# FluxML/Flux3D.jl

Hardware: AMD Instinct MI355X
Metric: chamfer_point_pairs_per_sec (higher is better)
Workload: dtype f32

## Files before the change

flux3d.jl_amd/csrc/chamfer.hip:

```cpp
#include <cmath>

#include "nn1_common.h"

using namespace fx3d;

#ifdef FX3D_PROBE
__device__ unsigned long long g_probe[4096 * 16];
#define FX3D_PROBE_MARK(k)                                                                   \
    do {                                                                                     \
        if (threadIdx.x == 0 && blockIdx.x < 4096) {                                         \
            g_probe[blockIdx.x * 16 + (k)] = __builtin_readcyclecounter();                   \
            if ((k) == 0) g_probe[blockIdx.x * 16 + 13] = wall_clock64();                    \
            if ((k) == 12) g_probe[blockIdx.x * 16 + 14] = wall_clock64();                   \
        }                                                                                    \
    } while (0)
__device__ unsigned long long g_probe2[256 * 16];
#define FX3D_PROBE_MARK2(k) do { if (threadIdx.x == 0 && blockIdx.x < 256) g_probe2[blockIdx.x * 16 + (k)] = __builtin_readcyclecounter(); } while (0)
__device__ unsigned long long g_probe3[16 * 16 * 8];
#define FX3D_PROBE_MARKW(k) do { if ((threadIdx.x & 63) == 0 && blockIdx.x < 16) g_probe3[(blockIdx.x * 16 + (threadIdx.x >> 6)) * 8 + (k)] = __builtin_readcyclecounter(); } while (0)
#else
#define FX3D_PROBE_MARK(k) do { } while (0)
#define FX3D_PROBE_MARK2(k) do { } while (0)
#define FX3D_PROBE_MARKW(k) do { } while (0)
#endif
// ... 53 lines not shown
    199, 198, 134, 135, 143, 142, 206, 207, 215, 223, 159, 151, 150, 158, 222, 214, 213, 221, 220, 212, 148, 156, 157, 149, 141, 205, 204, 140, 132, 196, 197, 133,
    69, 5, 4, 68, 76, 12, 13, 77, 85, 93, 92, 84, 20, 28, 29, 21, 22, 30, 94, 86, 87, 95, 31, 23, 15, 14, 78, 79, 71, 70, 6, 7,
};
constexpr size_t kHScratchBytes = (kHThreads / 64) * (32 * 8 + kHItemCap * 2 + 32 * 3 * 4) + 64 * 32;

__device__ __forceinline__ float vmin(float a, float b) {
    float r;
    asm("v_min_f32 %0, %1, %2" : "=v"(r) : "v"(a), "v"(b));
    return r;
}

__device__ __forceinline__ void split2h(float v, _Float16 &h, _Float16 &l) {
    h = (_Float16)v;
    l = (_Float16)(v - (float)h);
}

constexpr float kBetaC = 0x1.1p-18f;
constexpr float kBandB1 = 1.0f + 18.0f * kBetaC + 0x1p-20f;
constexpr float kBandA = 22.3f * kBetaC + 0x1p-19f;
__device__ __forceinline__ void make_pieces(float cx, float cy, float cz, h8 &p0, h8 &p1) {
    _Float16 hx, lx, hy, ly, hz, lz, n1, n2, n3;
    split2h(cx, hx, lx); split2h(cy, hy, ly); split2h(cz, hz, lz);
    const float n0 = ((cx * cx) + (cy * cy)) + (cz * cz);
    const float n = n0 + kBetaC * n0;
    n1 = (_Float16)n;
    const float r1 = n - (float)n1;
    n2 = (_Float16)r1;
    n3 = (_Float16)(r1 - (float)n2);
    const _Float16 z = (_Float16)0.0f;
    p0 = h8{hx, hx, lx, hy, hy, ly, hz, hz};
    p1 = h8{lz, n1, n2, n3, lx, ly, lz, z};
}

template <bool WANT_IDX, bool SPLITFUSE = false, bool PRUNE = false>
__global__ __launch_bounds__(kHThreads, 4) void nn1_f16_kernel(Nn1Params p) {
    extern __shared__ __attribute__((aligned(16))) float lds[];
    __shared__ __attribute__((aligned(16))) float red[4 * 4 * (kHThreads / 64) + 16];
    __shared__ int nfar[2];
    __shared__ unsigned short farlist[kHFarCap];
    constexpr int QB = (kHThreads / 64) * 32;

    const int L = blockIdx.x;
    const int per_cloud = p.tiles * p.nsplit;
    const bool by_xcd = 2 * p.B >= 8;
    const int slot = by_xcd ? L >> 3 : L;
    const int c = by_xcd ? (slot / per_cloud) * 8 + (L & 7) : slot / per_cloud;
    const int tile = (slot % per_cloud) / p.nsplit;
    const int split = (slot % per_cloud) % p.nsplit;
    if (c >= 2 * p.B) return;
    const int dir = c >= p.B ? 1 : 0;
    const int b = dir ? c - p.B : c;
    const int NQ = dir ? p.M : p.N;
    const int NC = dir ? p.N : p.M;
    if (tile >= (dir ? p.tiles_y : p.tiles_x)) return;
    if ((long long)split * p.chunk >= NC) return;
    const int ctail = (p.tail > 0 && p.nsplit == 1 && NC > p.chunk && NC - p.chunk <= p.tail) ? NC - p.chunk : 0;
    const int NCm = NC - ctail;
    const float *__restrict__ qb = (dir ? p.y : p.x) + (size_t)b * NQ * 3;
    const float *__restrict__ cb = (dir ? p.x : p.y) + (size_t)b * NC * 3;
    int32_t *idx_out = dir ? p.idx_y : p.idx_x;
    float *dmin_out = dir ? p.dmin_y : p.dmin_x;

    const int tid = threadIdx.x, lane = tid & 63;
    const int wv = __builtin_amdgcn_readfirstlane(tid >> 6);
    const int jq = lane & 31, hh = lane >> 5;
    const int CH = p.chunk;
    const int tpb = dir ? p.tpb_y : p.tpb;
    h8 *imgp = reinterpret_cast<h8 *>(lds);
    float4 *imgf = reinterpret_cast<float4 *>(lds);
    unsigned long long *wres = reinterpret_cast<unsigned long long *>(lds + 8 * (CH + 64));
    unsigned short *witems = reinterpret_cast<unsigned short *>(wres + (kHThreads / 64) * 32);
    float *wq = reinterpret_cast<float *>(witems + (kHThreads / 64) * kHItemCap);
    unsigned long long *qres = wres + wv * 32;
    unsigned short *items = witems + wv * kHItemCap;
    float *qtab = wq + wv * 96;
    const bool vec = (reinterpret_cast<uintptr_t>(cb) & 15) == 0;
    const bool one_shot = NCm <= CH;
    if (tid == 0) { nfar[0] = 0; nfar[1] = 0; }
    float qpre[3];
    {
        const int q0i = (tile * tpb) * QB + wv * 32 + jq;
        const int qc0 = q0i < NQ ? q0i : NQ - 1;
#pragma unroll
        for (int d = 0; d < 3; ++d) qpre[d] = qb[(size_t)qc0 * 3 + d];
    }
    if constexpr (PRUNE) {
        unsigned int *zc = reinterpret_cast<unsigned int *>(wres);
        for (int i = tid; i < 1040 + 16 * 256; i += kHThreads) zc[i] = 0u;
        int *gb = reinterpret_cast<int *>(wq + (kHThreads / 64) * 96) + 64 * 8;
        for (int i = tid; i < kHGroupsMax * 8; i += kHThreads) gb[i] = (i & 4) ? (int)0x80000000 : 0x7fffffff;
    }
    FX3D_PROBE_MARK(0);

    const bool own_chunk_only = p.nsplit > 1 && (long long)split * CH + (long long)p.nsplit * CH >= NCm;
    const int s_lo = own_chunk_only ? split * CH : 0;
    const int SN = own_chunk_only ? (NCm - s_lo < CH ? NCm - s_lo : CH) : NC;
    const float *__restrict__ sb = cb + (size_t)s_lo * 3;
    const bool parked = one_shot || own_chunk_only;
    float mu[3], cinf = 0.0f, varmax = 0.0f;
    float bxlo[3] = {0.f, 0.f, 0.f}, bxhi[3] = {0.f, 0.f, 0.f};
    bool allfin = true;
    {
        float mn[3] = {INFINITY, INFINITY, INFINITY}, mx[3] = {-INFINITY, -INFINITY, -INFINITY}, sm3[3] = {0.f, 0.f, 0.f};
        float sqt = 0.0f;
        const float pil[3] = {sb[0], sb[1], sb[2]};
        const int nsweep = (SN + kHThreads - 1) / kHThreads;
        for (int i0 = 0; i0 < nsweep; i0 += 4) {
            P3 v[4];
#pragma unroll
            for (int e = 0; e < 4; ++e) {
                const int pt = (i0 + e) * kHThreads + tid;
                v[e] = *reinterpret_cast<const P3 *>(sb + (size_t)(pt < SN ? pt : SN - 1) * 3);
            }
#pragma unroll
            for (int e = 0; e < 4; ++e) {
                const int pt = (i0 + e) * kHThreads + tid;
                mn[0] = fminf(mn[0], v[e].x); mx[0] = fmaxf(mx[0], v[e].x);
                mn[1] = fminf(mn[1], v[e].y); mx[1] = fmaxf(mx[1], v[e].y);
                mn[2] = fminf(mn[2], v[e].z); mx[2] = fmaxf(mx[2], v[e].z);
                if (pt < SN) {
                    sm3[0] = sm3[0] + v[e].x; sm3[1] = sm3[1] + v[e].y; sm3[2] = sm3[2] + v[e].z;
                    if (parked) imgf[((pt >> 5) * 2) * 32 + (pt & 31)] = float4{v[e].x, v[e].y, v[e].z, 0.0f};
                }
// ... 33 lines not shown
#undef NN1_ROW_SUM
            const float lo3[3] = {lo4.x, lo4.y, lo4.z}, hi3[3] = {hi4.x, hi4.y, hi4.z}, st3[3] = {st4.x, st4.y, st4.z};
            float m3[3], ci = 0.0f, vm = st4.w / fmaxf(0.25f * (float)SN, 1.0f);
            bool fin = true;
#pragma unroll
            for (int d = 0; d < 3; ++d) {
                const float lo = lo3[d], hi = hi3[d], st = st3[d];
                m3[d] = fminf(fmaxf(st / (float)SN, lo), hi);
                const float off = st / (float)SN - pil[d];
                vm = vm - off * off;
                ci = fmaxf(ci, fmaxf(hi - m3[d], m3[d] - lo));
                fin = fin && fabsf(st) < INFINITY;
            }
            if (lane == 0) {
                float4 *o4 = reinterpret_cast<float4 *>(red) + 4 * (kHThreads / 64);
                o4[0] = float4{m3[0], m3[1], m3[2], ci * 1.000001f};
                o4[1] = float4{vm, fin ? 1.0f : 0.0f, 0.0f, 0.0f};
                if (PRUNE) { o4[2] = float4{lo3[0], lo3[1], lo3[2], 0.0f}; o4[3] = float4{hi3[0], hi3[1], hi3[2], 0.0f}; }
            }
        }
        __syncthreads();
        {
            const float4 *o4 = reinterpret_cast<const float4 *>(red) + 4 * (kHThreads / 64);
            const float4 a = o4[0], b2 = o4[1];
            mu[0] = a.x; mu[1] = a.y; mu[2] = a.z; cinf = a.w;
            varmax = b2.x; allfin = b2.y != 0.0f;
            if (PRUNE) {
                const float4 l4 = o4[2], h4 = o4[3];
                bxlo[0] = l4.x; bxlo[1] = l4.y; bxlo[2] = l4.z; bxhi[0] = h4.x; bxhi[1] = h4.y; bxhi[2] = h4.z;
            }
        }
    }
    float rng = cinf;
    if (allfin && cinf < 1.0e16f && 3.0f * cinf * cinf > kRobustGate * varmax) {
        const float4 r = robust_range3<kHThreads, false>(sb, SN, parked, imgf, red, mu[0], mu[1], mu[2], cinf);
        mu[0] = r.x; mu[1] = r.y; mu[2] = r.z; rng = r.w;
    }
    const bool sane = allfin && cinf < 1.0e16f;
    float sc = 1.0f;
    if (sane && rng > 1.0e-30f) {
        int e;
        (void)frexpf(rng, &e);
        sc = ldexpf(1.0f, 7 - e);
    }
    auto uni = [](float v) { return __builtin_bit_cast(float, __builtin_amdgcn_readfirstlane(__builtin_bit_cast(int, v))); };
    mu[0] = uni(mu[0]); mu[1] = uni(mu[1]); mu[2] = uni(mu[2]); sc = uni(sc); rng = uni(rng); cinf = uni(cinf);
    const bool has_far = sane && rng < cinf;
    int fslot = 0;
    auto pieces = [&](float x, float y, float z, int pt, h8 &p0, h8 &p1) {
        const float sx = (x - mu[0]) * sc, sy = (y - mu[1]) * sc, sz = (z - mu[2]) * sc;
        if (!has_far) { make_pieces(sx, sy, sz, p0, p1); return; }
        const bool far = !(fmaxf(fmaxf(fabsf(sx), fabsf(sy)), fabsf(sz)) < 128.0f);
        make_pieces(far ? 0.f : sx, far ? 0.f : sy, far ? 0.f : sz, p0, p1);
        if (far) {
            p1[7] = (_Float16)kPadF16;
            const int f = atomicAdd(&nfar[fslot], 1);
            if (f < kHFarCap) farlist[f] = (unsigned short)pt;
        }
    };

    [[maybe_unused]] float4 *cs = nullptr, *qsw = nullptr;
    [[maybe_unused]] bool sorted_c = false;
    [[maybe_unused]] int qwlen = 0;
    [[maybe_unused]] float4 *boxes = nullptr;
    if constexpr (PRUNE) {
        cs = p.pscr + (size_t)blockIdx.x * p.pscr_stride;
        qsw = cs + kHChunkMax;
        boxes = reinterpret_cast<float4 *>(wq + (kHThreads / 64) * 96);
        unsigned int *ccnt = reinterpret_cast<unsigned int *>(wres);
        unsigned int *qtot = ccnt + 520;
        unsigned int *qwh = qtot + 520;
        const bool last_t = tile == (dir ? p.tiles_y : p.tiles_x) - 1;
        const int qw0 = tile * tpb * QB;
        const int qw1 = last_t || qw0 + tpb * QB > NQ ? NQ : qw0 + tpb * QB;
        qwlen = qw1 - qw0;
        const int cnt = NCm;
        const bool do_sort = sane && cnt >= 512;
        const bool sorted_q = do_sort && NQ <= 4 * kHThreads;
        P3 qv[4];
        if (sorted_q) {
#pragma unroll
            for (int e = 0; e < 4; ++e) {
                const int qp = 256 * wv + 64 * e + lane;
                qv[e] = *reinterpret_cast<const P3 *>(qb + (size_t)(qp < NQ ? qp : NQ - 1) * 3);
            }
        }
        FX3D_PROBE_MARK2(0);
        int *gbox = reinterpret_cast<int *>(boxes + 64 * 2);
        auto group_box = [&](int wrow, float x, float y, float z) {
            int *g = gbox + (wrow >> 5) * 8;
            atomicMin(g + 0, fkey((x - mu[0]) * sc)); atomicMin(g + 1, fkey((y - mu[1]) * sc)); atomicMin(g + 2, fkey((z - mu[2]) * sc));
            atomicMax(g + 4, fkey((x - mu[0]) * sc)); atomicMax(g + 5, fkey((y - mu[1]) * sc)); atomicMax(g + 6, fkey((z - mu[2]) * sc));
        };
        if (do_sort) {
            float4 cv[4];
#pragma unroll
            for (int e = 0; e < 4; ++e) {
                const int pt = e * kHThreads + tid;
                cv[e] = float4{0.f, 0.f, 0.f, 0.f};
                if (pt < cnt) cv[e] = imgf[((pt >> 5) * 2) * 32 + (pt & 31)];
            }
            FX3D_PROBE_MARK2(1);
            float inv[3], off[3], cfl[3], cfh[3];
#pragma unroll
            for (int d = 0; d < 3; ++d) {
                const float fr = has_far ? 0.125f * rng : 128.0f / sc;
                const float flo = fmaxf(bxlo[d], mu[d] - fr), fhi = fminf(bxhi[d], mu[d] + fr);
                inv[d] = fhi > flo ? 8.0f / (fhi - flo) : 0.0f;
                off[d] = -flo * inv[d];
                cfl[d] = flo; cfh[d] = fhi;
            }
            auto cell = [&](float x, float y, float z) -> unsigned int {
                const unsigned int ux = (unsigned int)(int)fminf(fmaxf(__builtin_fmaf(x, inv[0], off[0]), 0.0f), 7.0f);
                const unsigned int uy = (unsigned int)(int)fminf(fmaxf(__builtin_fmaf(y, inv[1], off[1]), 0.0f), 7.0f);
                const unsigned int uz = (unsigned int)(int)fminf(fmaxf(__builtin_fmaf(z, inv[2], off[2]), 0.0f), 7.0f);
                return ux | (uy << 3) | (uz << 6);
            };

            unsigned int ccr[4], qcr[4];
            auto count_cells = [&](bool valid, unsigned int t, auto &&add) -> unsigned int {
                unsigned int rank = 0u;
                bool mine = valid;
                const unsigned int tn = (unsigned int)__builtin_amdgcn_update_dpp((int)~t, (int)t, 0x111, 0xF, 0xF, false);
                if (__builtin_popcountll(__ballot(valid && t == tn)) >= 8) {
                    unsigned long long rem = __ballot(valid);
                    for (int it = 0; it < 12 && rem; ++it) {
                        const unsigned int t0 = (unsigned int)__builtin_amdgcn_readlane((int)t, __builtin_ctzll(rem));
                        const unsigned long long grp = __ballot(mine && t == t0);
                        rem &= ~grp;
                        if (__builtin_popcountll(grp) < 4) continue;
                        unsigned int base = 0u;
                        if ((int)lane == __builtin_ctzll(grp)) base = add(t0, (unsigned int)__builtin_popcountll(grp));
                        base = (unsigned int)__builtin_amdgcn_readlane((int)base, __builtin_ctzll(grp));
                        if (mine && t == t0) {
                            rank = base + __builtin_amdgcn_mbcnt_hi((unsigned int)(grp >> 32), __builtin_amdgcn_mbcnt_lo((unsigned int)grp, 0u));
                            mine = false;
                        }
                    }
                }
                if (mine) rank = add(t, 1u);
                return rank;
            };
#pragma unroll
            for (int e = 0; e < 4; ++e) {
                const int pt = e * kHThreads + tid;
                const unsigned int t = pt < cnt ? cell(cv[e].x, cv[e].y, cv[e].z) : 0u;
                ccr[e] = (t << 16) | count_cells(pt < cnt, t, [&](unsigned int c, unsigned int n) { return atomicAdd(&ccnt[c], n); });
            }
            int *qbb = reinterpret_cast<int *>(boxes + 64 * 2 + kHGroupsMax * 2 - 2);
            if (sorted_q) {
                int kl[3] = {0x7fffffff, 0x7fffffff, 0x7fffffff}, kh[3] = {(int)0x80000000, (int)0x80000000, (int)0x80000000};
#pragma unroll
                for (int e = 0; e < 4; ++e) {
                    const int qp = 256 * wv + 64 * e + lane;
                    if (qp < NQ) {
                        const int k3[3] = {fkey(qv[e].x), fkey(qv[e].y), fkey(qv[e].z)};
#pragma unroll
                        for (int d = 0; d < 3; ++d) { kl[d] = kl[d] < k3[d] ? kl[d] : k3[d]; kh[d] = kh[d] > k3[d] ? kh[d] : k3[d]; }
                    }
                }
#pragma unroll
                for (int d = 0; d < 3; ++d) {
                    int a = row_mm_key<false>(kl[d]), b2 = row_mm_key<true>(kh[d]);
                    a = imm<false>(a, dpp_keepi<0x142, 0xA>(a)); a = imm<false>(a, dpp_keepi<0x143, 0xC>(a));
                    b2 = imm<true>(b2, dpp_keepi<0x142, 0xA>(b2)); b2 = imm<true>(b2, dpp_keepi<0x143, 0xC>(b2));
                    if (lane == 63) { atomicMin(qbb + d, a); atomicMax(qbb + 4 + d, b2); }
                }
            }
            FX3D_PROBE_MARK2(2);
            __syncthreads();
            FX3D_PROBE_MARK2(3);
            float qinv[3] = {0.f, 0.f, 0.f}, qoff[3] = {0.f, 0.f, 0.f};
            if (sorted_q) {
                const float ext = fmaxf(fmaxf(cfh[0] - cfl[0], cfh[1] - cfl[1]), cfh[2] - cfl[2]);
#pragma unroll
// ... 86 lines not shown
                            group_box(rank - qw0, qv[e].x, qv[e].y, qv[e].z);
                        }
                    }
                }
            }
        }
        if (!sorted_q) {
            for (int q0 = qw0 + wv * 64; q0 < qw1; q0 += kHThreads) {
                const int qp = q0 + lane;
                const P3 r = *reinterpret_cast<const P3 *>(qb + (size_t)(qp < qw1 ? qp : qw1 - 1) * 3);
                if (qp < qw1) qsw[qp - qw0] = float4{r.x, r.y, r.z, __builtin_bit_cast(float, qp)};
                const int kx = fkey((r.x - mu[0]) * sc), ky = fkey((r.y - mu[1]) * sc), kz = fkey((r.z - mu[2]) * sc);
                const int lx = row_mm_key<false>(kx), ly = row_mm_key<false>(ky), lz = row_mm_key<false>(kz);
                const int hx = row_mm_key<true>(kx), hy = row_mm_key<true>(ky), hz = row_mm_key<true>(kz);
                if ((lane & 15) == 0 && qp < qw1) {
                    int *g = gbox + ((qp - qw0) >> 5) * 8;
                    atomicMin(g + 0, lx); atomicMin(g + 1, ly); atomicMin(g + 2, lz);
                    atomicMax(g + 4, hx); atomicMax(g + 5, hy); atomicMax(g + 6, hz);
                }
            }
        }
        FX3D_PROBE_MARK2(8);
    }
    FX3D_PROBE_MARK(1);

    const float cm2 = 3.0f * (fminf(cinf * sc, 128.0f) * fminf(cinf * sc, 128.0f));
    float qr[3], da = 0.0f;
    float da_far = 0.0f;
    [[maybe_unused]] float dpr = INFINITY;
    bool qfin = true;
    int qi = 0;
    bool qok = true;
    h8 bq;
    double acc = 0.0;

    const int jfirst = split * CH, jstep = p.nsplit * CH;
    for (int j0 = jfirst; j0 < NCm; j0 += jstep) {
        const int cnt = (NCm - j0) < CH ? (NCm - j0) : CH;
        const int cnt_pad = (cnt + 32 * kHLT - 1) / (32 * kHLT) * (32 * kHLT);
        if (j0 > jfirst) __syncthreads();
        if constexpr (PRUNE) {
            for (int tl = tid >> 4; tl * 64 < cnt_pad + 64; tl += kHThreads / 16) {
                float4 r4[4];
#pragma unroll
                for (int k = 0; k < 4; ++k) {
                    const int pt = tl * 64 + k * 16 + (tid & 15);
                    r4[k] = float4{0.f, 0.f, 0.f, 0.f};
                    if (pt < cnt) r4[k] = imgf[((pt >> 5) * 2) * 32 + (pt & 31)];
                }
                float lo3[3] = {INFINITY, INFINITY, INFINITY}, hi3[3] = {-INFINITY, -INFINITY, -INFINITY};
#pragma unroll
                for (int k = 0; k < 4; ++k) {
                    const int pt = tl * 64 + k * 16 + (tid & 15), i0 = ((pt >> 5) * 2) * 32 + (pt & 31);
                    h8 p0, p1;
                    if (pt < cnt) {
                        pieces(r4[k].x, r4[k].y, r4[k].z, pt, p0, p1);
                        const int id = sorted_c ? __builtin_bit_cast(int, r4[k].w) : j0 + pt;
                        cs[pt] = float4{r4[k].x, r4[k].y, r4[k].z, __builtin_bit_cast(float, id)};
                        const float b3[3] = {(r4[k].x - mu[0]) * sc, (r4[k].y - mu[1]) * sc, (r4[k].z - mu[2]) * sc};
#pragma unroll
                        for (int d = 0; d < 3; ++d) { lo3[d] = vmin(lo3[d], b3[d]); hi3[d] = -vmin(-hi3[d], -b3[d]); }
                    } else {
                        make_pieces(0.f, 0.f, 0.f, p0, p1);
                        p1[7] = (_Float16)kPadF16;
                    }
                    imgp[i0] = p0;
                    imgp[i0 + 32] = p1;
                }
                float bl[3], bh[3];
#pragma unroll
// ... 632 lines not shown
        }
        const float dd = __builtin_bit_cast(float, (unsigned int)(r >> 32));
        int32_t *idx_out = dir ? p.idx_y : p.idx_x;
        float *dmin_out = dir ? p.dmin_y : p.dmin_x;
        if (idx_out) idx_out[(size_t)b * NQ + qi] = (int)(unsigned int)r;
        if (dmin_out) dmin_out[(size_t)b * NQ + qi] = dd;
        acc = (double)dd;
    }
    if (p.partials) {
        __shared__ double sm[kThreads / 64];
        const double tot = block_sum<kThreads>(acc, sm);
        if (!p.ticket) {
            if (threadIdx.x == 0) p.partials[(size_t)c * tiles_f + blockIdx.x] = tot;
            return;
        }
        if (threadIdx.x < 64) {
            const FinalizeArgs fa{reinterpret_cast<unsigned long long *>(p.partials), p.ticket, p.nvalid, p.B, tiles_f, p.tiles_x, p.tiles_y,
                                  p.sums_out, p.loss_out, p.N, p.M, p.Bg, p.w1, p.w2};
            (void)fused_finalize_wave0(fa, (size_t)c * tiles_f + blockIdx.x, tot, (int)threadIdx.x);
        }
    }
}

}

namespace fx3d {

size_t nn1_f16_lds_bytes(int chunk) { return (size_t)chunk * 8 * sizeof(float) + kHScratchBytes; }

constexpr size_t kHBoxBytes = 64 * 2 * sizeof(float4) + kHGroupsMax * 32;

template <bool WANT_IDX>
static fx3d_status launch_f16(const Nn1Params &p, int grid, size_t lds_bytes, hipStream_t st) {
    void (*const kfn)(Nn1Params) = p.pscr ? &nn1_f16_kernel<WANT_IDX, false, true>
                                   : p.fuse_split ? &nn1_f16_kernel<WANT_IDX, true> : &nn1_f16_kernel<WANT_IDX, false>;
    const size_t box = p.pscr ? kHBoxBytes : 0;
    const fx3d_status arc = ensure_dynamic_lds(reinterpret_cast<const void *>(kfn), (int)(nn1_f16_lds_bytes(kHChunkMax) + box), "nn1_f16_kernel");
    if (arc != FX3D_OK) return arc;
    hipLaunchKernelGGL(kfn, dim3(grid), dim3(kHThreads), lds_bytes + box, st, p);
    FX3D_LAUNCH_CHECK();
    return FX3D_OK;
}

fx3d_status nn1_f16_launch(const Nn1Params &p, int grid, size_t lds_bytes, hipStream_t st) {
    return p.idx_x || p.idx_y ? launch_f16<true>(p, grid, lds_bytes, st) : launch_f16<false>(p, grid, lds_bytes, st);
}

fx3d_status nn1_split_finalize_launch(const Nn1Params &p, int tiles_f, hipStream_t st) {
    hipLaunchKernelGGL(nn1_split_finalize_kernel, dim3(tiles_f, 2 * p.B), dim3(kThreads), 0, st, p, tiles_f);
    FX3D_LAUNCH_CHECK();
    return FX3D_OK;
}

}
```

flux3d.jl_amd/csrc/chamfer_host.hip:

```cpp
#include <cmath>
#include <cstdlib>

#include "nn1_common.h"

using namespace fx3d;

namespace {

struct FinalizeParams {
    const double *partials;
    int B, tiles, tiles_x, tiles_y;
    double *sums;
    float *loss;
    int N, M, D;
    long long Bg;
    float w1, w2;
};

__global__ __launch_bounds__(kThreads) void chamfer_finalize_partials_kernel(FinalizeParams f) {
    __shared__ double sm[kThreads / 64];
    double tot[2];
    for (int dir = 0; dir < 2; ++dir) {
        const int nt = dir ? f.tiles_y : f.tiles_x;
        const long long n = (long long)f.B * nt;
// ... 174 lines not shown
    if (plan_kernel(pl, D) != NN1_F16 || pl.nsplit != 1 || pl.tail != 0 || maxc > pl.chunk || maxc < 1024 || !opt(OPT_NN1_PRUNE)) return 0;
    if ((pl.tpb > pl.tpb_y ? pl.tpb : pl.tpb_y) * 16 + 2 > kHGroupsMax - 1) return 0;
    if ((pl.tpb < pl.tpb_y ? pl.tpb : pl.tpb_y) < 2) return 0;
    return kHChunkMax + (pl.tpb > pl.tpb_y ? pl.tpb : pl.tpb_y) * 512 + kHTail;
}

struct Workspace {
    int tiles;
    size_t sums, gres, need, pscr, total;
};
Workspace workspace_layout(const Plan &pl, int N, int M, int B, int D) {
    Workspace w{};
    const int maxq = N > M ? N : M;
    w.tiles = pl.nsplit > 1 ? ceil_div(maxq, kThreads) : pl.tiles;
    w.sums = (size_t)2 * B * w.tiles * sizeof(double);
    w.gres = w.sums + 2 * sizeof(double);
    w.need = w.gres + (pl.nsplit > 1 ? (size_t)pl.nsplit * 2 * B * maxq * sizeof(unsigned long long) : 0);
    w.pscr = (w.need + 255) & ~(size_t)255;
    const size_t ps = (size_t)prune_rows_per_block(pl, N, M, D) * pl.grid * sizeof(float4);
    w.total = ps ? w.pscr + ps : w.need;
    return w;
}

constexpr long long kSplitFuseMax = 255;

fx3d_status run_nn1(Nn1Params p, int D, const Plan &pl, hipStream_t st) {
    p.tiles = pl.tiles; p.tiles_x = pl.tiles_x; p.tiles_y = pl.tiles_y; p.chunk = pl.chunk;
    p.tpb = pl.tpb; p.tpb_y = pl.tpb_y;
    p.tail = pl.tail;
    p.nsplit = p.gres ? pl.nsplit : 1;
    p.fuse_split = p.gres && p.ticket ? 1 : 0;
    p.pscr_stride = p.pscr ? prune_rows_per_block(pl, p.N, p.M, D) : 0;
    if (!p.pscr_stride) p.pscr = nullptr;
    const Nn1Kernel k = plan_kernel(pl, D);
    ProfileScope prof("nn1", st);
    if (k == NN1_F16) return nn1_f16_launch(p, pl.grid, pl.lds_bytes, st);
    return nn1_exact_launch(k, p, D, pl.R, pl.grid, pl.lds_bytes, st);
}

}

namespace fx3d {

fx3d_status chamfer_check_shapes(const char *fn, const void *x, int N, const void *y, int M, int B, int D) {
    FX3D_REQUIRE(x && y, "%s: null input pointer", fn);
    FX3D_REQUIRE(N > 0 && M > 0 && B > 0 && D > 0, "%s: empty input (N=%d M=%d B=%d D=%d)", fn, N, M, B, D);
    FX3D_REQUIRE((long long)B * 2 * (((long long)(N > M ? N : M) + 255) / 256) < (1ll << 30),
                 "%s: problem too large for one launch", fn);
    return FX3D_OK;
}

fx3d_status chamfer_forward(const float *x, int N, const float *y, int M, int B, int D, double *sums_dev, float *loss_dev,
                            long long Bg, float w1, float w2, int32_t *idx_x, int32_t *idx_y, void *ws, size_t ws_bytes,
                            hipStream_t st, const char *fn) {
    fx3d_status rc = chamfer_check_shapes(fn, x, N, y, M, B, D);
    if (rc) return rc;
    const Plan pl = make_plan(N, M, B, D);
    const Workspace w = workspace_layout(pl, N, M, B, D);
    if (!ws || ws_bytes < w.need) {
        set_error("%s: workspace too small (%zu < %zu bytes)", fn, ws ? ws_bytes : (size_t)0, w.need);
        return FX3D_ERR_WORKSPACE;
    }
    char *const base = static_cast<char *>(ws);
    Nn1Params p{};
    p.x = x; p.y = y; p.N = N; p.M = M; p.B = B;
    p.idx_x = idx_x; p.idx_y = idx_y;
// ... 113 lines not shown
```

flux3d.jl_amd/csrc/nn1_common.h:

```cpp
#pragma once
#include "fx3d_common.h"

namespace fx3d {

constexpr int kThreads = 256;
constexpr int kTile = 32;
constexpr int kChunkMax = 4096;

struct Nn1Params {
    const float *x;
    const float *y;
    int N, M, B;
    int32_t *idx_x, *idx_y;
    float *dmin_x, *dmin_y;
    double *partials;
    int tiles;
    int tiles_x, tiles_y;
    int chunk;
    int tpb;
    int tpb_y;
    unsigned int *ticket;
    unsigned int nvalid;
    double *sums_out;
    float *loss_out;
    float w1, w2;
    long long Bg;
    int nsplit;
    unsigned long long *gres;
    int qstride;
    int fuse_split;
    int tail;
    float4 *pscr;
    int pscr_stride;
};

enum Nn1Kernel { NN1_GENERIC, NN1_SMALL_D, NN1_TINY, NN1_F16 };
fx3d_status nn1_exact_launch(Nn1Kernel k, const Nn1Params &p, int D, int R, int grid, size_t lds_bytes, hipStream_t st);
size_t nn1_f16_lds_bytes(int chunk);
fx3d_status nn1_f16_launch(const Nn1Params &p, int grid, size_t lds_bytes, hipStream_t st);
fx3d_status nn1_split_finalize_launch(const Nn1Params &p, int tiles_f, hipStream_t st);

__device__ __forceinline__ float min3f(float a, float b, float c) {
    return __builtin_fminf(__builtin_fminf(a, b), c);
}

template <int DIM>
__device__ __forceinline__ float sqd(const float (&q)[DIM], const float (&c)[DIM]) {
    float t0 = q[0] - c[0];
    float s = t0 * t0;
#pragma unroll
    for (int d = 1; d < DIM; ++d) {
        float t = q[d] - c[d];
        s = s + t * t;
    }
    return s;
}

__device__ __forceinline__ bool fless(float a, float b) { return (a < b) || (b != b && a == a); }
__device__ __forceinline__ unsigned int dist_key(float d) { return d != d ? 0x7fc00000u : __builtin_bit_cast(unsigned int, d); }

template <int DIM>
__device__ __forceinline__ void nn1_scan_isless(const float (&q)[DIM], const float *__restrict__ cb, int NC, float &best, int &bi) {
    float c0[DIM];
#pragma unroll
    for (int d = 0; d < DIM; ++d) c0[d] = cb[d];
    best = sqd<DIM>(q, c0);
    bi = 0;
    for (int j = 1; j < NC; ++j) {
        float cc[DIM];
#pragma unroll
        for (int d = 0; d < DIM; ++d) cc[d] = cb[(size_t)j * DIM + d];
        const float dd = sqd<DIM>(q, cc);
        if (fless(dd, best)) { best = dd; bi = j; }
    }
}

constexpr int kHThreads = 1024;
#ifndef FX3D_HLT
#define FX3D_HLT 2
#endif
constexpr int kHLT = FX3D_HLT;
constexpr int kHChunkMax = 4096;
constexpr int kHTail = 64;
constexpr int kHGroupsMax = 8 * 16 + 2 + 1;

constexpr int kTyThreads = 256;
constexpr int kTyQ = 16;
constexpr int kTySl = 16;
constexpr int kTyG = 16;

__device__ __forceinline__ float chamfer_loss_from_sums(double sa, double sb, int N, int M, int D,
                                                        long long Bg, float w1, float w2) {
    const float dA = (float)(sa / ((double)D * (double)N * (double)Bg)) * 3.0f;
    const float dB = (float)(sb / ((double)D * (double)M * (double)Bg)) * 3.0f;
    return (w1 * dA) + (w2 * dB);
}

#if defined(__HIP_DEVICE_COMPILE__) && !defined(__gfx950__)
#error "nn1_common.h: the relaxed-atomic + s_waitcnt hand-off between blocks is validated on gfx950 only (see the note above)"
#endif
struct FinalizeArgs {
    unsigned long long *pp;
    unsigned int *ticket;
    unsigned int nvalid;
    int B, stride, tiles_x, tiles_y;
    double *sums_out;
    float *loss_out;
    int N, M;
    long long Bg;
    float w1, w2;
};
__device__ __forceinline__ int fused_finalize_wave0(const FinalizeArgs &f, size_t slot, double tot, int lane) {
    int last = 0;
    if (lane == 0) {
        __hip_atomic_store(&f.pp[slot], __builtin_bit_cast(unsigned long long, tot), __ATOMIC_RELAXED, __HIP_MEMORY_SCOPE_AGENT);
        asm volatile("s_waitcnt vmcnt(0)" ::: "memory");
        const unsigned int old = __hip_atomic_fetch_add(f.ticket, 1u, __ATOMIC_RELAXED, __HIP_MEMORY_SCOPE_AGENT);
// ... 34 lines not shown
```

Before: 14590 billion.

## Add uniform-grid spatial hash fast path for pruned nearest-neighbor search

Adds a GRID variant of the pruned f16 kernel. For compact, well-conditioned single-chunk clouds it bins the candidate points into a G^3 uniform grid in LDS using a counting sort. Each query then searches the 27 neighboring cells, and expands rings with a provable distance bound for queries that are not yet resolved. When the grid checks fail or too many queries remain unresolved, it falls back to the existing sort/box-prune path. This trades brute-force tiled distance evaluation for data-dependent exact search, with added complexity, scalar-divergent ring loops, and extra synchronisations.

New measurement: 18920 billion (median of 6 runs). 29.7% higher.

```diff
diff --git a/flux3d.jl_amd/csrc/chamfer.hip b/flux3d.jl_amd/csrc/chamfer.hip
--- a/flux3d.jl_amd/csrc/chamfer.hip
+++ b/flux3d.jl_amd/csrc/chamfer.hip
@@ -109,12 +109,15 @@
     p1 = h8{lz, n1, n2, n3, lx, ly, lz, z};
 }
 
-template <bool WANT_IDX, bool SPLITFUSE = false, bool PRUNE = false>
+template <bool WANT_IDX, bool SPLITFUSE = false, bool PRUNE = false, bool GRID = false>
 __global__ __launch_bounds__(kHThreads, 4) void nn1_f16_kernel(Nn1Params p) {
     extern __shared__ __attribute__((aligned(16))) float lds[];
     __shared__ __attribute__((aligned(16))) float red[4 * 4 * (kHThreads / 64) + 16];
     __shared__ int nfar[2];
     __shared__ unsigned short farlist[kHFarCap];
+    __shared__ int gflag;
+    __shared__ unsigned int gocc;
+    __shared__ unsigned int gunf;
     constexpr int QB = (kHThreads / 64) * 32;
 
     const int L = blockIdx.x;
@@ -161,11 +164,22 @@
 #pragma unroll
         for (int d = 0; d < 3; ++d) qpre[d] = qb[(size_t)qc0 * 3 + d];
     }
+    [[maybe_unused]] int gG = kGridMinG;
     if constexpr (PRUNE) {
         unsigned int *zc = reinterpret_cast<unsigned int *>(wres);
         for (int i = tid; i < 1040 + 16 * 256; i += kHThreads) zc[i] = 0u;
         int *gb = reinterpret_cast<int *>(wq + (kHThreads / 64) * 96) + 64 * 8;
         for (int i = tid; i < kHGroupsMax * 8; i += kHThreads) gb[i] = (i & 4) ? (int)0x80000000 : 0x7fffffff;
+        if constexpr (GRID) if (p.grid) {
+            while (gG < kGridMaxG && kGridPpc * (gG + 1) * (gG + 1) * (gG + 1) <= NCm) ++gG;
+            unsigned int *gz = reinterpret_cast<unsigned int *>(lds) + ((NCm + 63) >> 6) * 256 + 128;
+            if (NCm >= kGridMinCand) {
+                const int i4 = 4 * tid;
+                if (i4 < gG * gG * gG + 4) *reinterpret_cast<uint4 *>(&gz[i4 + (i4 & ~127)]) = uint4{0u, 0u, 0u, 0u};
+                if (tid == 0 && gG == kGridMaxG) *reinterpret_cast<uint4 *>(&gz[2 * 4096]) = uint4{0u, 0u, 0u, 0u};
+            }
+            if (tid == 0) { gflag = 0; gocc = 0u; gunf = 0u; }
+        }
     }
     FX3D_PROBE_MARK(0);
 
@@ -265,9 +279,11 @@
         }
     }
     float rng = cinf;
+    [[maybe_unused]] bool robust_ran = false;
     if (allfin && cinf < 1.0e16f && 3.0f * cinf * cinf > kRobustGate * varmax) {
         const float4 r = robust_range3<kHThreads, false>(sb, SN, parked, imgf, red, mu[0], mu[1], mu[2], cinf);
         mu[0] = r.x; mu[1] = r.y; mu[2] = r.z; rng = r.w;
+        robust_ran = true;
     }
     const bool sane = allfin && cinf < 1.0e16f;
     float sc = 1.0f;
@@ -292,11 +308,300 @@
         }
     };
 
+    [[maybe_unused]] auto count_cells = [&](bool valid, unsigned int t, auto &&add) -> unsigned int {
+        unsigned int rank = 0u;
+        bool mine = valid;
+        const unsigned int tn = (unsigned int)__builtin_amdgcn_update_dpp((int)~t, (int)t, 0x111, 0xF, 0xF, false);
+        if (__builtin_popcountll(__ballot(valid && t == tn)) >= 8) {
+            unsigned long long rem = __ballot(valid);
+            for (int it = 0; it < 12 && rem; ++it) {
+                const unsigned int t0 = (unsigned int)__builtin_amdgcn_readlane((int)t, __builtin_ctzll(rem));
+                const unsigned long long grp = __ballot(mine && t == t0);
+                rem &= ~grp;
+                if (__builtin_popcountll(grp) < 4) continue;
+                unsigned int base = 0u;
+                if ((int)lane == __builtin_ctzll(grp)) base = add(t0, (unsigned int)__builtin_popcountll(grp));
+                base = (unsigned int)__builtin_amdgcn_readlane((int)base, __builtin_ctzll(grp));
+                if (mine && t == t0) {
+                    rank = base + __builtin_amdgcn_mbcnt_hi((unsigned int)(grp >> 32), __builtin_amdgcn_mbcnt_lo((unsigned int)grp, 0u));
+                    mine = false;
+                }
+            }
+        }
+        if (mine) rank = add(t, 1u);
+        return rank;
+    };
+    [[maybe_unused]] bool grid_done = false;
+    [[maybe_unused]] double gacc = 0.0;
+    [[maybe_unused]] float4 gcv[4];
+    [[maybe_unused]] P3 gqv[4];
+    [[maybe_unused]] bool gpre = false, gabandon = false;
+    if constexpr (PRUNE && GRID) {
+        bool gtry = p.grid && NQ <= 4 * kHThreads && sane && !has_far && !robust_ran && one_shot && NCm >= kGridMinCand &&
+                    3.0f * cinf * cinf <= kGridScreen * varmax;
+        const int cnt = NCm, G = gG, ncell = G * G * G;
+        float ginv[3], goff[3], gwid[3];
+#pragma unroll
+        for (int d = 0; d < 3; ++d) {
+            const float lo = uni(bxlo[d]), ext = uni(bxhi[d]) - lo;
+            const bool ok = ext > 1.0e-30f;
+            ginv[d] = ok ? (float)G / ext : 0.0f;
+            goff[d] = -lo * ginv[d];
+            gwid[d] = ext / (float)G;
+            gtry = gtry && ok;
+        }
+        {
+            const float e0 = uni(bxhi[0]) - uni(bxlo[0]), e1 = uni(bxhi[1]) - uni(bxlo[1]), e2 = uni(bxhi[2]) - uni(bxlo[2]);
+            gtry = gtry && fmaxf(fmaxf(e0, e1), e2) <= kGridMaxAspect * fminf(fminf(e0, e1), e2);
+        }
+        if (gtry) {
+#pragma unroll
+            for (int e = 0; e < 4; ++e) {
+                const int qp = 256 * wv + 64 * e + lane;
+                gqv[e] = *reinterpret_cast<const P3 *>(qb + (size_t)(qp < NQ ? qp : NQ - 1) * 3);
+            }
+            unsigned int *gc = reinterpret_cast<unsigned int *>(lds) + ((cnt + 63) >> 6) * 256 + 128;
+            auto gwd = [](unsigned int t) { return t + (t & ~127u); };
+            const float gm1 = (float)(G - 1);
+            auto gcoord = [&](float t) -> int { return (int)fminf(fmaxf(t, 0.0f), gm1); };
+            const bool last_t = tile == (dir ? p.tiles_y : p.tiles_x) - 1;
+            const int qw0 = tile * tpb * QB;
+            const int qw1 = last_t || qw0 + tpb * QB > NQ ? NQ : qw0 + tpb * QB;
+            unsigned int gcr[4];
+#pragma unroll
+            for (int e = 0; e < 4; ++e) {
+                const int pt = e * kHThreads + tid;
+                gcv[e] = float4{0.f, 0.f, 0.f, 0.f};
+                if (pt < cnt) gcv[e] = imgf[((pt >> 5) * 2) * 32 + (pt & 31)];
+            }
+            gpre = true;
+            bool gbad = false;
+            unsigned int nocc = 0u;
+#pragma unroll
+            for (int e = 0; e < 4; ++e) {
+                const int pt = e * kHThreads + tid;
+                unsigned int t = 0u;
+                if (pt < cnt)
+                    t = (unsigned int)gcoord(__builtin_fmaf(gcv[e].x, ginv[0], goff[0])) +
+                        (unsigned int)G * ((unsigned int)gcoord(__builtin_fmaf(gcv[e].y, ginv[1], goff[1])) + (unsigned int)G * (unsigned int)gcoord(__builtin_fmaf(gcv[e].z, ginv[2], goff[2])));
+                const unsigned int rank = count_cells(pt < cnt, t, [&](unsigned int c, unsigned int n) { return atomicAdd(&gc[gwd(c)], n); });
+                gbad = gbad || rank >= kGridCap;
+                nocc += (unsigned int)__builtin_popcountll(__ballot(pt < cnt && rank == 0u));
+                gcr[e] = (t << 16) | rank;
+            }
+            if (lane == 0) atomicAdd(&gocc, nocc);
+            {
+                auto qcheck = [&](const P3 &q) {
+                    const float t3[3] = {__builtin_fmaf(q.x, ginv[0], goff[0]), __builtin_fmaf(q.y, ginv[1], goff[1]), __builtin_fmaf(q.z, ginv[2], goff[2])};
+#pragma unroll
+                    for (int d = 0; d < 3; ++d) gbad = gbad || !(t3[d] >= -kGridQueryMargin && t3[d] <= (float)G + kGridQueryMargin);
+                };
+#pragma unroll
+                for (int e = 0; e < 4; ++e) qcheck(gqv[e]);
+                if (__ballot(gbad) && lane == 0) gflag = 1;
+            }
+            FX3D_PROBE_MARK2(1);
+            __syncthreads();
+            const bool fast = __builtin_amdgcn_readfirstlane(gflag) == 0 && 100u * (unsigned int)__builtin_amdgcn_readfirstlane((int)gocc) >= kGridMinOccPct * (unsigned int)ncell;
+            if (fast) {
+            const bool own = 4 * tid <= ncell;
+            uint4 c4 = uint4{0u, 0u, 0u, 0u};
+            if (own) c4 = *reinterpret_cast<const uint4 *>(&gc[gwd(4u * (unsigned int)tid)]);
+            const unsigned int tot = (c4.x + c4.y) + (c4.z + c4.w);
+            int inci = (int)tot;
+            inci += __builtin_amdgcn_update_dpp(0, inci, 0x111, 0xF, 0xF, true);
+            inci += __builtin_amdgcn_update_dpp(0, inci, 0x112, 0xF, 0xF, true);
+            inci += __builtin_amdgcn_update_dpp(0, inci, 0x114, 0xF, 0xF, true);
+            inci += __builtin_amdgcn_update_dpp(0, inci, 0x118, 0xF, 0xF, true);
+            inci += __builtin_amdgcn_update_dpp(0, inci, 0x142, 0xA, 0xF, false);
+            inci += __builtin_amdgcn_update_dpp(0, inci, 0x143, 0xC, 0xF, false);
+            const unsigned int inc = (unsigned int)inci;
+            unsigned int *wtot = reinterpret_cast<unsigned int *>(red);
+            if (lane == 63) wtot[wv] = inc;
+            FX3D_PROBE_MARK2(2);
+            __syncthreads();
+            {
+                unsigned int pre = 0u;
+                {
+                    const uint4 *t4 = reinterpret_cast<const uint4 *>(wtot);
+                    const uint4 a0 = t4[0], a1 = t4[1], a2 = t4[2], a3 = t4[3];
+                    const unsigned int tw[16] = {a0.x, a0.y, a0.z, a0.w, a1.x, a1.y, a1.z, a1.w, a2.x, a2.y, a2.z, a2.w, a3.x, a3.y, a3.z, a3.w};
+#pragma unroll
+                    for (int w = 0; w < 16; ++w) pre += w < wv ? tw[w] : 0u;
+                }
+                const unsigned int s0 = pre + inc - tot;
+                if (own) *reinterpret_cast<uint4 *>(&gc[gwd(4u * (unsigned int)tid)]) = uint4{s0, s0 + c4.x, s0 + c4.x + c4.y, s0 + c4.x + c4.y + c4.z};
+                if (ncell == 4 * kHThreads && tid == 0) gc[gwd((unsigned int)ncell)] = (unsigned int)cnt;
+                FX3D_PROBE_MARK2(3);
+                __syncthreads();
+                float4 *rows = reinterpret_cast<float4 *>(lds);
+#pragma unroll
+                for (int e = 0; e < 4; ++e) {
+                    const int pt = e * kHThreads + tid;
+                    if (pt < cnt) rows[gc[gwd(gcr[e] >> 16)] + (gcr[e] & 0xffffu)] = float4{gcv[e].x, gcv[e].y, gcv[e].z, __builtin_bit_cast(float, pt)};
+                }
+                if (tid == 0) p.pscr[(size_t)blockIdx.x * p.pscr_stride] = float4{0.f, 0.f, 0.f, __builtin_bit_cast(float, kGridMarker)};
+                FX3D_PROBE_MARK2(4);
+                __syncthreads();
+                for (int q0 = qw0; q0 < qw1; q0 += kHThreads) {
+                    const int qp = q0 + tid;
+                    const P3 q = *reinterpret_cast<const P3 *>(qb + (size_t)(qp < qw1 ? qp : qw1 - 1) * 3);
+                    const float tq[3] = {__builtin_fmaf(q.x, ginv[0], goff[0]), __builtin_fmaf(q.y, ginv[1], goff[1]), __builtin_fmaf(q.z, ginv[2], goff[2])};
+                    int iq[3];
+                    float er[3];
+#pragma unroll
+                    for (int d = 0; d < 3; ++d) { iq[d] = gcoord(tq[d]); er[d] = 0x1p-20f * ((float)G + fabsf(tq[d])); }
+                    unsigned long long best = ~0ull;
+                    auto eval = [&](unsigned int j) {
+                        const float4 r = rows[j];
+                        const float dx = q.x - r.x, dy = q.y - r.y, dz = q.z - r.z;
+                        const float dd = ((dx * dx) + dy * dy) + dz * dz;
+                        const unsigned long long key = ((unsigned long long)__builtin_bit_cast(unsigned int, dd) << 32) | __builtin_bit_cast(unsigned int, r.w);
+                        best = key < best ? key : best;
+                    };
+                    {
+                        const int x0 = iq[0] > 0 ? iq[0] - 1 : 0, x1 = iq[0] < G - 1 ? iq[0] + 1 : G - 1;
+                        unsigned int rs[9], re[9];
+#pragma unroll
+                        for (int k = 0; k < 9; ++k) {
+                            const int y = iq[1] + k % 3 - 1, z = iq[2] + k / 3 - 1;
+                            const bool ok = (unsigned int)y < (unsigned int)G && (unsigned int)z < (unsigned int)G;
+                            const int base = ((ok ? z : iq[2]) * G + (ok ? y : iq[1])) * G;
+                            rs[k] = gc[gwd((unsigned int)(base + x0))];
+                            re[k] = gc[gwd((unsigned int)(base + x1 + 1))];
+                            if (!ok) re[k] = rs[k];
+                        }
+#pragma unroll
+                        for (int k = 0; k < 9; ++k)
+                            for (unsigned int j = rs[k]; j < re[k]; ++j) eval(j);
+                    }
+                    auto bound2 = [&](int r) -> float {
+                        float lb = INFINITY;
+#pragma unroll
+                        for (int d = 0; d < 3; ++d) {
+                            const int hi = iq[d] + r + 1, lo = iq[d] - r;
+                            if (hi <= G - 1) lb = fminf(lb, (((float)hi - tq[d]) - er[d]) * gwid[d]);
+                            if (lo >= 1) lb = fminf(lb, ((tq[d] - (float)lo) - er[d]) * gwid[d]);
+                        }
+                        lb = fmaxf(lb, 0.0f);
+                        return (lb * lb) * (1.0f - 0x1p-10f);
+                    };
+                    const float l21 = bound2(1), bd1 = __builtin_bit_cast(float, (unsigned int)(best >> 32));
+                    bool done = bd1 < l21 && l21 >= 0x1p-100f;
+                    if (q0 == qw0) {
+                        const unsigned int nun = (unsigned int)__builtin_popcountll(__ballot(!(bd1 <= 4.0f * l21) && qp < qw1));
+                        if (lane == 0 && nun) atomicAdd(&gunf, nun);
+                        __syncthreads();
+                        const unsigned int nq = (unsigned int)(qw1 - qw0 < kHThreads ? qw1 - qw0 : kHThreads);
+                        if (kGridMaxFar * (unsigned int)__builtin_amdgcn_readfirstlane((int)gunf) > nq) { gabandon = true; break; }
+                    }
+                    auto wave_min_key = [](unsigned long long mine) -> unsigned long long {
+                        auto wmin = [](int k) {
+                            k = row_mm_key<false>(k);
+                            const int a = __builtin_amdgcn_readlane(k, 0), b2 = __builtin_amdgcn_readlane(k, 16), c2 = __builtin_amdgcn_readlane(k, 32), d2 = __builtin_amdgcn_readlane(k, 48);
+                            return imm<false>(imm<false>(a, b2), imm<false>(c2, d2));
+                        };
+                        const unsigned int hi = (unsigned int)(mine >> 32);
+                        const int kd = hi < 0x7fffffffu ? (int)hi : 0x7fffffff;
+                        const int dmin = wmin(kd);
+                        const int imin = wmin(kd == dmin ? (int)(unsigned int)mine : 0x7fffffff);
+                        return dmin != 0x7fffffff ? ((unsigned long long)(unsigned int)dmin << 32) | (unsigned int)imin : ~0ull;
+                    };
+                    for (unsigned long long todo = __ballot(!done && qp < qw1); todo; todo &= todo - 1ull) {
+                        const int l = __builtin_ctzll(todo);
+                        auto bl = [&](float v) { return __builtin_bit_cast(float, __builtin_amdgcn_readlane(__builtin_bit_cast(int, v), l)); };
+                        const float sq[3] = {bl(q.x), bl(q.y), bl(q.z)}, stq[3] = {bl(tq[0]), bl(tq[1]), bl(tq[2])}, ser[3] = {bl(er[0]), bl(er[1]), bl(er[2])};
+                        const int siq[3] = {__builtin_amdgcn_readlane(iq[0], l), __builtin_amdgcn_readlane(iq[1], l), __builtin_amdgcn_readlane(iq[2], l)};
+                        unsigned long long kb = ((unsigned long long)(unsigned int)__builtin_amdgcn_readlane((int)(unsigned int)(best >> 32), l) << 32) |
+                                                (unsigned int)__builtin_amdgcn_readlane((int)(unsigned int)best, l);
+                        for (int r = 2; r < G; ++r) {
+                            if (r > kGridMaxRing) {
+                                unsigned long long mine = ~0ull;
+                                for (int j = lane; j < cnt; j += 64) {
+                                    const float4 r4 = rows[j];
+                                    const float dx = sq[0] - r4.x, dy = sq[1] - r4.y, dz = sq[2] - r4.z;
+                                    const float dd = ((dx * dx) + dy * dy) + dz * dz;
+                                    const unsigned long long key = ((unsigned long long)__builtin_bit_cast(unsigned int, dd) << 32) | __builtin_bit_cast(unsigned int, r4.w);
+                                    mine = key < mine ? key : mine;
+                                }
+                                kb = wave_min_key(mine);
+                                break;
+                            }
+                            int c0[3], n[3];
+#pragma unroll
+                            for (int d = 0; d < 3; ++d) {
+                                c0[d] = siq[d] - r > 0 ? siq[d] - r : 0;
+                                n[d] = (siq[d] + r < G - 1 ? siq[d] + r : G - 1) - c0[d] + 1;
+                            }
+                            const int ncube = n[0] * n[1] * n[2];
+                            const float rx = 1.0f / (float)n[0], ry = 1.0f / (float)n[1];
+                            const float bdist = __builtin_bit_cast(float, (unsigned int)(kb >> 32));
+                            unsigned long long mine = ~0ull;
+                            for (int c = lane; c < ncube; c += 64) {
+                                const int cyz = (int)(((float)c + 0.5f) * rx), uz = (int)(((float)cyz + 0.5f) * ry);
+                                const int cc[3] = {c0[0] + (c - cyz * n[0]), c0[1] + (cyz - uz * n[1]), c0[2] + uz};
+                                float g2 = 0.0f;
+#pragma unroll
+                                for (int d = 0; d < 3; ++d) {
+                                    const int k = cc[d] - siq[d];
+                                    const float g = k > 0 ? ((float)cc[d] - stq[d]) - ser[d] : k < 0 ? (stq[d] - (float)(cc[d] + 1)) - ser[d] : 0.0f;
+                                    const float gw = fmaxf(g * gwid[d], 0.0f);
+                                    g2 = g2 + gw * gw;
+                                }
+                                if (g2 * (1.0f - 0x1p-10f) > bdist) continue;
+                                const unsigned int cell = (unsigned int)((cc[2] * G + cc[1]) * G + cc[0]);
+                                const unsigned int js = gc[gwd(cell)], je = gc[gwd(cell + 1u)];
+                                for (unsigned int j = js; j < je; ++j) {
+                                    const float4 r4 = rows[j];
+                                    const float dx = sq[0] - r4.x, dy = sq[1] - r4.y, dz = sq[2] - r4.z;
+                                    const float dd = ((dx * dx) + dy * dy) + dz * dz;
+                                    const unsigned long long key = ((unsigned long long)__builtin_bit_cast(unsigned int, dd) << 32) | __builtin_bit_cast(unsigned int, r4.w);
+                                    mine = key < mine ? key : mine;
+                                }
+                            }
+                            mine = wave_min_key(mine);
+                            kb = mine < kb ? mine : kb;
+                            float lb = INFINITY;
+#pragma unroll
+                            for (int d = 0; d < 3; ++d) {
+                                const int hi = siq[d] + r + 1, lo = siq[d] - r;
+                                if (hi <= G - 1) lb = fminf(lb, (((float)hi - stq[d]) - ser[d]) * gwid[d]);
+                                if (lo >= 1) lb = fminf(lb, ((stq[d] - (float)lo) - ser[d]) * gwid[d]);
+                            }
+                            lb = fmaxf(lb, 0.0f);
+                            const float l2 = (lb * lb) * (1.0f - 0x1p-10f);
+                            if (__builtin_bit_cast(float, (unsigned int)(kb >> 32)) < l2 && l2 >= 0x1p-100f) break;
+                        }
+                        if (lane == l) best = kb;
+                    }
+                    if (qp < qw1) {
+                        const float dd = __builtin_bit_cast(float, (unsigned int)(best >> 32));
+                        if (WANT_IDX && idx_out) idx_out[(size_t)b * NQ + qp] = (int)(unsigned int)best;
+                        if (dmin_out) dmin_out[(size_t)b * NQ + qp] = dd;
+                        gacc += (double)dd;
+                    }
+                }
+                if (gabandon) {
+#pragma unroll
+                    for (int e = 0; e < 4; ++e) {
+                        const int pt = e * kHThreads + tid;
+                        if (pt < cnt) imgf[((pt >> 5) * 2) * 32 + (pt & 31)] = float4{gcv[e].x, gcv[e].y, gcv[e].z, 0.0f};
+                    }
+                    gacc = 0.0;
+                } else {
+                FX3D_PROBE_MARK2(5);
+                grid_done = true;
+                }
+            }
+            }
+        }
+    }
+
     [[maybe_unused]] float4 *cs = nullptr, *qsw = nullptr;
     [[maybe_unused]] bool sorted_c = false;
     [[maybe_unused]] int qwlen = 0;
     [[maybe_unused]] float4 *boxes = nullptr;
-    if constexpr (PRUNE) {
+    if constexpr (PRUNE) if (!grid_done) {
         cs = p.pscr + (size_t)blockIdx.x * p.pscr_stride;
         qsw = cs + kHChunkMax;
         boxes = reinterpret_cast<float4 *>(wq + (kHThreads / 64) * 96);
@@ -309,13 +614,14 @@
         qwlen = qw1 - qw0;
         const int cnt = NCm;
         const bool do_sort = sane && cnt >= 512;
-        const bool sorted_q = do_sort && NQ <= 4 * kHThreads;
+        const bool sorted_q = do_sort && NQ <= 4 * kHThreads && !gabandon;
         P3 qv[4];
         if (sorted_q) {
 #pragma unroll
             for (int e = 0; e < 4; ++e) {
                 const int qp = 256 * wv + 64 * e + lane;
-                qv[e] = *reinterpret_cast<const P3 *>(qb + (size_t)(qp < NQ ? qp : NQ - 1) * 3);
+                if (gpre) qv[e] = gqv[e];
+                else qv[e] = *reinterpret_cast<const P3 *>(qb + (size_t)(qp < NQ ? qp : NQ - 1) * 3);
             }
         }
         FX3D_PROBE_MARK2(0);
@@ -331,7 +637,8 @@
             for (int e = 0; e < 4; ++e) {
                 const int pt = e * kHThreads + tid;
                 cv[e] = float4{0.f, 0.f, 0.f, 0.f};
-                if (pt < cnt) cv[e] = imgf[((pt >> 5) * 2) * 32 + (pt & 31)];
+                if (gpre) cv[e] = gcv[e];
+                else if (pt < cnt) cv[e] = imgf[((pt >> 5) * 2) * 32 + (pt & 31)];
             }
             FX3D_PROBE_MARK2(1);
             float inv[3], off[3], cfl[3], cfh[3];
@@ -351,29 +658,6 @@
             };
 
             unsigned int ccr[4], qcr[4];
-            auto count_cells = [&](bool valid, unsigned int t, auto &&add) -> unsigned int {
-                unsigned int rank = 0u;
-                bool mine = valid;
-                const unsigned int tn = (unsigned int)__builtin_amdgcn_update_dpp((int)~t, (int)t, 0x111, 0xF, 0xF, false);
-                if (__builtin_popcountll(__ballot(valid && t == tn)) >= 8) {
-                    unsigned long long rem = __ballot(valid);
-                    for (int it = 0; it < 12 && rem; ++it) {
-                        const unsigned int t0 = (unsigned int)__builtin_amdgcn_readlane((int)t, __builtin_ctzll(rem));
-                        const unsigned long long grp = __ballot(mine && t == t0);
-                        rem &= ~grp;
-                        if (__builtin_popcountll(grp) < 4) continue;
-                        unsigned int base = 0u;
-                        if ((int)lane == __builtin_ctzll(grp)) base = add(t0, (unsigned int)__builtin_popcountll(grp));
-                        base = (unsigned int)__builtin_amdgcn_readlane((int)base, __builtin_ctzll(grp));
-                        if (mine && t == t0) {
-                            rank = base + __builtin_amdgcn_mbcnt_hi((unsigned int)(grp >> 32), __builtin_amdgcn_mbcnt_lo((unsigned int)grp, 0u));
-                            mine = false;
-                        }
-                    }
-                }
-                if (mine) rank = add(t, 1u);
-                return rank;
-            };
 #pragma unroll
             for (int e = 0; e < 4; ++e) {
                 const int pt = e * kHThreads + tid;
@@ -526,10 +810,10 @@
     int qi = 0;
     bool qok = true;
     h8 bq;
-    double acc = 0.0;
+    double acc = gacc;
 
     const int jfirst = split * CH, jstep = p.nsplit * CH;
-    for (int j0 = jfirst; j0 < NCm; j0 += jstep) {
+    for (int j0 = jfirst; j0 < NCm && !grid_done; j0 += jstep) {
         const int cnt = (NCm - j0) < CH ? (NCm - j0) : CH;
         const int cnt_pad = (cnt + 32 * kHLT - 1) / (32 * kHLT) * (32 * kHLT);
         if (j0 > jfirst) __syncthreads();
@@ -1228,7 +1512,7 @@
 
 template <bool WANT_IDX>
 static fx3d_status launch_f16(const Nn1Params &p, int grid, size_t lds_bytes, hipStream_t st) {
-    void (*const kfn)(Nn1Params) = p.pscr ? &nn1_f16_kernel<WANT_IDX, false, true>
+    void (*const kfn)(Nn1Params) = p.pscr ? (p.grid ? &nn1_f16_kernel<WANT_IDX, false, true, true> : &nn1_f16_kernel<WANT_IDX, false, true>)
                                    : p.fuse_split ? &nn1_f16_kernel<WANT_IDX, true> : &nn1_f16_kernel<WANT_IDX, false>;
     const size_t box = p.pscr ? kHBoxBytes : 0;
     const fx3d_status arc = ensure_dynamic_lds(reinterpret_cast<const void *>(kfn), (int)(nn1_f16_lds_bytes(kHChunkMax) + box), "nn1_f16_kernel");
diff --git a/flux3d.jl_amd/csrc/chamfer_host.hip b/flux3d.jl_amd/csrc/chamfer_host.hip
--- a/flux3d.jl_amd/csrc/chamfer_host.hip
+++ b/flux3d.jl_amd/csrc/chamfer_host.hip
@@ -230,6 +230,7 @@
     p.fuse_split = p.gres && p.ticket ? 1 : 0;
     p.pscr_stride = p.pscr ? prune_rows_per_block(pl, p.N, p.M, D) : 0;
     if (!p.pscr_stride) p.pscr = nullptr;
+    p.grid = p.pscr && opt(OPT_NN1_PRUNE) == 1 && (p.N > p.M ? p.N : p.M) >= kGridMinCand ? 1 : 0;
     const Nn1Kernel k = plan_kernel(pl, D);
     ProfileScope prof("nn1", st);
     if (k == NN1_F16) return nn1_f16_launch(p, pl.grid, pl.lds_bytes, st);
diff --git a/flux3d.jl_amd/csrc/nn1_common.h b/flux3d.jl_amd/csrc/nn1_common.h
--- a/flux3d.jl_amd/csrc/nn1_common.h
+++ b/flux3d.jl_amd/csrc/nn1_common.h
@@ -32,6 +32,7 @@
     int tail;
     float4 *pscr;
     int pscr_stride;
+    int grid;
 };
 
 enum Nn1Kernel { NN1_GENERIC, NN1_SMALL_D, NN1_TINY, NN1_F16 };
@@ -83,6 +84,18 @@
 constexpr int kHChunkMax = 4096;
 constexpr int kHTail = 64;
 constexpr int kHGroupsMax = 8 * 16 + 2 + 1;
+
+constexpr int kGridPpc = 1;
+constexpr int kGridMinG = 8, kGridMaxG = 16;
+constexpr int kGridMinCand = 2048;
+constexpr unsigned int kGridCap = 16;
+constexpr float kGridScreen = 6.0f;
+constexpr unsigned int kGridMinOccPct = 45;
+constexpr float kGridMaxAspect = 1.5f;
+constexpr unsigned int kGridMaxFar = 16;
+constexpr int kGridMaxRing = 3;
+constexpr float kGridQueryMargin = 0.5f;
+constexpr unsigned int kGridMarker = 0x47524944u;
 
 constexpr int kTyThreads = 256;
 constexpr int kTyQ = 16;
```
